# LCJebe/PCReg

Hardware: AMD Instinct MI355X
Metric: KNN Gpairs/s end-to-end (search + filters + RANSAC per step; registrations/s = 1000/ms_per_step) (higher is better)
Workload: dtype f32 (search: f16-split matrix-core candidates, exact f32 re-rank) / f64 (RANSAC)

## Files before the change

pcreg_amd/csrc/api.hip:

```cpp
#include "common.hpp"
#include <atomic>
#include <cstdarg>
#include <cmath>
#include <mutex>
#include <algorithm>
#include <vector>

namespace pcreg {

static thread_local char g_err[512] = "no error";
void set_error(const char* fmt, ...) {
    va_list ap; va_start(ap, fmt);
    vsnprintf(g_err, sizeof g_err, fmt, ap);
    va_end(ap);
}

constexpr int kKnnMaxK = PCREG_KNN_MAX_K;
constexpr int kKnnMaxQ = 4 << 20;
constexpr int kRangeMaxQ = 4 << 20;
constexpr int kScoreMaxQ = 4 << 20;
static std::mutex g_mu;
static int g_device_ok = -1;
static hipStream_t g_stream = nullptr;

// ... 39 lines not shown

}

using namespace pcreg;

#define GUARD()                                                     \
    std::lock_guard<std::mutex> lock__(g_mu);                       \
    do { int rc__ = ensure_device(); if (rc__) return rc__; } while (0)
#define TRY(expr) do { int rc__ = (expr); if (rc__) return rc__; } while (0)

namespace pcreg {
static std::atomic<int> g_debug[kDbgCount];
int debug_flag(DebugKey k) { return g_debug[k].load(std::memory_order_relaxed); }
struct Counters { DebugKey key; int n; unsigned long long* dev; };
static Counters g_match_stats{kDbgMatchStats, 8, nullptr}, g_knn_stats{kDbgKnnStats, 6, nullptr}, g_ransac_stats{kDbgRansacStats, 3, nullptr},
                g_cluster_stats{kDbgClusterStats, 4, nullptr}, g_desc_stats{kDbgDescStats, 10, nullptr},
                g_knn_direct_stats{kDbgKnnDirectStats, 3, nullptr};
static unsigned long long* counters_dev(Counters& c) {
    if (!debug_flag(c.key)) return nullptr;
    if (!c.dev) {
        if (hipMalloc((void**)&c.dev, c.n * sizeof(unsigned long long)) != hipSuccess) { c.dev = nullptr; return nullptr; }
        (void)hipMemset(c.dev, 0, c.n * sizeof(unsigned long long));
    }
    return c.dev;
}
static int counters_read(const Counters& c, long long* out, int reset, int first = 0, int count = -1) {
    PCREG_ARG(out != nullptr);
    if (count < 0) count = c.n - first;
    for (int k = 0; k < count; ++k) out[k] = 0;
    if (!c.dev) return PCREG_OK;
    PCREG_HIP(hipDeviceSynchronize());
    unsigned long long h[8];
    PCREG_HIP(hipMemcpy(h, c.dev + first, count * sizeof h[0], hipMemcpyDeviceToHost));
    for (int k = 0; k < count; ++k) out[k] = (long long)h[k];
    if (reset) PCREG_HIP(hipMemset(c.dev + first, 0, count * sizeof h[0]));
    return PCREG_OK;
}
unsigned long long* match_stats_dev() { return counters_dev(g_match_stats); }
unsigned long long* knn_stats_dev() { return counters_dev(g_knn_stats); }
unsigned long long* ransac_stats_dev() { return counters_dev(g_ransac_stats); }
unsigned long long* cluster_stats_dev() { return counters_dev(g_cluster_stats); }
unsigned long long* desc_stats_dev() { return counters_dev(g_desc_stats); }
unsigned long long* knn_direct_stats_dev() { return counters_dev(g_knn_direct_stats); }
}

extern "C" {

int pcreg_debug_set(const char* key, int value) {
    static const char* const names[pcreg::kDbgCount] = {"knn_exact", "match_exact", "match_force_fallback", "ransac_fused", "ransac_nolane",
                                                        "ransac_f64score", "ransac_resident_f64", "align_times", "align_shape", "seg_debug",
                                                        "seg_batched", "seg_wave_finalize", "match_stats", "final_batch_mb", "knn_nocull",
                                                        "knn_stats", "ransac_pass2", "ransac_stats", "range_sort_cap", "cluster_noskip",
                                                        "cluster_stats", "knn_tail_cap", "score_batch_slots", "fpfh_radius_lanes", "desc_stats",
                                                        "knn_direct", "knn_direct_stats"};
    PCREG_ARG(key != nullptr);
    for (int k = 0; k < pcreg::kDbgCount; ++k)
        if (!strcmp(key, names[k])) { pcreg::g_debug[k].store(value, std::memory_order_relaxed); return PCREG_OK; }
    pcreg::set_error("pcreg_debug_set: unknown key '%s'", key);
    return PCREG_E_ARG;
}

int pcreg_debug_match_stats(long long out[8], int reset) { return pcreg::counters_read(pcreg::g_match_stats, out, reset); }
int pcreg_debug_knn_stats(long long out[4], int reset) { return pcreg::counters_read(pcreg::g_knn_stats, out, reset, 0, 4); }
int pcreg_debug_knn_unit_stats(long long out[2], int reset) { return pcreg::counters_read(pcreg::g_knn_stats, out, reset, 4, 2); }
int pcreg_debug_knn_direct_stats(long long out[3], int reset) { return pcreg::counters_read(pcreg::g_knn_direct_stats, out, reset); }
int pcreg_debug_ransac_stats(long long out[3], int reset) { return pcreg::counters_read(pcreg::g_ransac_stats, out, reset); }
int pcreg_debug_cluster_stats(long long out[4], int reset) { return pcreg::counters_read(pcreg::g_cluster_stats, out, reset); }
int pcreg_debug_desc_stats(long long out[10], int reset) {
    PCREG_ARG(out != nullptr);
    TRY(pcreg::counters_read(pcreg::g_desc_stats, out, reset, 0, 8));
    return pcreg::counters_read(pcreg::g_desc_stats, out + 8, reset, 8, 2);
}

const char* pcreg_last_error(void) { return g_err; }
const char* pcreg_version(void) { return "pcreg-hip 0.1 (gfx950)"; }

int pcreg_device_count(int* count) {
    PCREG_ARG(count != nullptr);
    hipError_t e = hipGetDeviceCount(count);
    if (e != hipSuccess) { *count = 0; (void)hipGetLastError(); }
    return PCREG_OK;
}

static void*  g_pin[2] = {nullptr, nullptr};
static size_t g_pin_bytes[2] = {0, 0};
static hipEvent_t g_pairs_ev = nullptr;

int pcreg_set_device(int ordinal) {
    std::lock_guard<std::mutex> lock(g_mu);
    int count = 0;
    if (hipGetDeviceCount(&count) != hipSuccess || count <= 0) { set_error("no HIP device available"); (void)hipGetLastError(); return PCREG_E_NODEVICE; }
    PCREG_ARG(ordinal >= 0 && ordinal < count);
    scratch().release_all();
    if (g_stream) { (void)hipStreamDestroy(g_stream); g_stream = nullptr; }
    if (g_pairs_ev) { (void)hipEventDestroy(g_pairs_ev); g_pairs_ev = nullptr; }
    for (int k = 0; k < 2; ++k) if (g_pin[k]) { (void)hipHostFree(g_pin[k]); g_pin[k] = nullptr; g_pin_bytes[k] = 0; }
    g_device_ok = -1;
    PCREG_HIP(hipSetDevice(ordinal));
    return ensure_device();
}

int pcreg_device_name(char* buf, int cap) {
    PCREG_ARG(buf != nullptr && cap > 0);
    GUARD();
    int dev = 0; PCREG_HIP(hipGetDevice(&dev));
    hipDeviceProp_t prop; PCREG_HIP(hipGetDeviceProperties(&prop, dev));
    snprintf(buf, (size_t)cap, "%s (%s, %d CUs)", prop.name, prop.gcnArchName, prop.multiProcessorCount);
// ... 2416 lines not shown
```

pcreg_amd/csrc/common.hpp:

```cpp
#pragma once
#include <cstdlib>
#include <hip/hip_runtime.h>
#include <cstdint>
#include <cstdio>
#include <cstring>
#include <algorithm>
#include <string>
#include "../../include/pcreg.h"

namespace pcreg {

void set_error(const char* fmt, ...);
int  ensure_device();

#define PCREG_HIP(call)                                                                  \
    do {                                                                                 \
        hipError_t e__ = (call);                                                         \
        if (e__ != hipSuccess) {                                                         \
            ::pcreg::set_error("%s failed: %s (%s:%d)", #call, hipGetErrorString(e__),   \
                               __FILE__, __LINE__);                                      \
            return PCREG_E_HIP;                                                          \
        }                                                                                \
    } while (0)

// ... 2 lines not shown
        if (!(cond)) {                                                                   \
            ::pcreg::set_error("bad argument: %s (%s:%d)", #cond, __FILE__, __LINE__);   \
            return PCREG_E_ARG;                                                          \
        }                                                                                \
    } while (0)

struct Scratch {
    static constexpr int kSlots = 24;
    void*  ptr[kSlots]  = {};
    size_t size[kSlots] = {};
    int get(int slot, size_t bytes, void** out);
    void release_all();
};
Scratch& scratch();
struct Stage {
    Scratch& s; int next = 0;
    template <class T> int take(size_t count, T** out) {
        void* p = nullptr;
        const int rc = s.get(next, count * sizeof(T), &p);
        if (rc == PCREG_OK) ++next;
        *out = (T*)p;
        return rc;
    }
};

enum DebugKey {
    kDbgKnnExact = 0,
    kDbgMatchExact,
    kDbgMatchForceFallback,
    kDbgRansacFused,
    kDbgRansacNoLane,
    kDbgRansacF64Score,
    kDbgRansacResidentF64,
    kDbgAlignTimes,
    kDbgAlignShape,
    kDbgSegDebug,
    kDbgSegBatched,
    kDbgSegWaveFinalize,
    kDbgMatchStats,
    kDbgFinalBatchMB,
    kDbgKnnNoCull,
    kDbgKnnStats,
    kDbgRansacPass2,
    kDbgRansacStats,
    kDbgRangeSortCap,
    kDbgClusterNoSkip,
    kDbgClusterStats,
    kDbgKnnTailCap,
    kDbgScoreBatchSlots,
    kDbgFpfhRadiusLanes,
    kDbgDescStats,
    kDbgKnnDirect,
    kDbgKnnDirectStats,
    kDbgCount
};
int debug_flag(DebugKey k);
unsigned long long* match_stats_dev();
unsigned long long* knn_stats_dev();
unsigned long long* knn_direct_stats_dev();
unsigned long long* ransac_stats_dev();
unsigned long long* cluster_stats_dev();
unsigned long long* desc_stats_dev();
#ifdef PCREG_EXPERIMENTS
static inline int pcreg_env_int(const char* name, int dflt) { const char* e = getenv(name); return e ? atoi(e) : dflt; }
static inline const char* pcreg_env_str(const char* name) { return getenv(name); }
#define PCREG_EXP_ENV(name, dflt) pcreg_env_int(name, dflt)
#define PCREG_EXP_STR(name) pcreg_env_str(name)
#else
#define PCREG_EXP_ENV(name, dflt) (dflt)
#define PCREG_EXP_STR(name) ((const char*)nullptr)
#endif

static inline size_t align_up(size_t x, size_t a) { return (x + a - 1) / a * a; }

struct WsWalk {
    char* base; size_t off = 0;
    explicit WsWalk(void* b) : base((char*)b) {}
    void* take_bytes(size_t bytes) { void* p = base ? base + off : nullptr; off += bytes; return p; }
    template <class T> T* take(size_t count, size_t align = 256) { return (T*)take_bytes(align_up(count * sizeof(T), align)); }
    size_t bytes() const { return off; }
};

template <typename T>
static int upload_cols(const T* host, int n, int ld, int cols, T* dev, hipStream_t st) {
    if (n <= 0 || cols <= 0) return PCREG_OK;
    if (ld == n) { PCREG_HIP(hipMemcpyAsync(dev, host, sizeof(T) * (size_t)n * cols, hipMemcpyHostToDevice, st)); }
    else PCREG_HIP(hipMemcpy2DAsync(dev, sizeof(T) * (size_t)n, host, sizeof(T) * (size_t)ld, sizeof(T) * (size_t)n, cols, hipMemcpyHostToDevice, st));
    return PCREG_OK;
}

struct RansacDims { int n_cap; int iters; int B; };

size_t ransac_workspace_bytes(int iters, int B, int n_cap);
int launch_ransac(const double* p1, const double* p2, int ld, const int32_t* offsets ,
                  const int32_t* n_dev , int n_cap, int B,
                  const pcreg_ransac_opts& o, const int32_t* sample_idx_dev,
                  pcreg_dev_ransac_result* out , int32_t* inlier_idx, int32_t* iter_inl ,
                  int32_t* iter_inl_ref, void* ws, size_t ws_bytes, hipStream_t st);
int launch_ransac_partial(const double* p1, const double* p2, int ld, const int32_t* n_dev, int n_cap,
                          const pcreg_ransac_opts& o, const int32_t* sample_idx_dev, int hyp_begin, int hyp_count,
                          pcreg_dev_ransac_part* part, void* ws, size_t ws_bytes, hipStream_t st);
int launch_ransac_finish(const double* p1, const double* p2, int ld, const int32_t* n_dev, int n_cap,
                         const pcreg_ransac_opts& o, const pcreg_dev_ransac_part* combined,
                         pcreg_dev_ransac_result* out, int32_t* inlier_idx, hipStream_t st, int n_parts = 1);
int launch_estimate_transform(const double* p1, const double* p2, int n, int ld, double* T16_dev,
                              int32_t* empty_dev, hipStream_t st);
// ... 185 lines not shown
```

pcreg_amd/csrc/knn_fast.hip:

```cpp
#include "common.hpp"
#include "select.hpp"
#include "knn_fast_common.hpp"
#include <cmath>
#include <cstdlib>
#include <cstdio>
#include <algorithm>

namespace pcreg {

size_t knn_f16_prep_bytes(int M);
void knn_f16_shape(int Q, int M, int target_blocks, int* q_blocks, int* W);
int launch_prep_model_f16(const float* m, int M, int ldm, const void* prep, unsigned* rm2, void* mtiles, int32_t* seed_cnt,
                          void* seed_slots, hipStream_t st);
int launch_knn_candidates_f16(const float* q, int Q, int ldq, const int32_t* qperm, const float* dk, int M, const void* prep,
                              const void* mtiles, const float* tbox, const float* ubox, int cull, int32_t* n_vis, int32_t* vis_list, uint32_t* vis_mask, unsigned* gthr,
                              void* cand_ent, int32_t* cand_cnt, void* ctr, int target_blocks, bool dry, bool timed, const float* ug_part,
                              int ug_nparts, int ug_cells, void* ug_prep, int* W_out, hipStream_t st);

namespace {

__global__ __launch_bounds__(kBlock) void model_bbox_partial_kernel(const float* __restrict__ m, int M, int ldm,
                                                                    float* __restrict__ part ,
                                                                    int32_t* __restrict__ zero_me, int n_zero) {
    for (int i = blockIdx.x * kBlock + threadIdx.x; i < n_zero; i += gridDim.x * kBlock) zero_me[i] = 0;
// ... 97 lines not shown
__global__ __launch_bounds__(kBlock) void model_order_scatter_kernel(const float* __restrict__ m, int M, int ldm, const Prep* __restrict__ prep,
                                                                     int32_t* __restrict__ off, int32_t* __restrict__ perm, float* __restrict__ ms) {
    for (int i = blockIdx.x * kBlock + threadIdx.x; i < M; i += gridDim.x * kBlock) {
        const float x = m[i], y = m[i + (size_t)ldm], z = m[i + 2 * (size_t)ldm];
        const int d = atomicAdd(&off[sort_key(x, y, z, prep)], 1);
        perm[d] = i; ms[d] = x; ms[d + (size_t)M] = y; ms[d + 2 * (size_t)M] = z;
    }
}
__global__ __launch_bounds__(kBlock) void tile_box_kernel(const float* __restrict__ ms, int M, float* __restrict__ tbox, float* __restrict__ ubox) {
    float lo[3] = {INFINITY, INFINITY, INFINITY}, hi[3] = {-INFINITY, -INFINITY, -INFINITY};
    for (int r = threadIdx.x; r < kT16; r += kBlock) {
        const int i = blockIdx.x * kT16 + r;
        float ulo[3] = {INFINITY, INFINITY, INFINITY}, uhi[3] = {-INFINITY, -INFINITY, -INFINITY};
        if (i < M) {
#pragma unroll
            for (int c = 0; c < 3; ++c) { ulo[c] = uhi[c] = ms[i + (size_t)c * M]; lo[c] = fminf(lo[c], ulo[c]); hi[c] = fmaxf(hi[c], uhi[c]); }
        }
#pragma unroll
        for (int c = 0; c < 3; ++c) {
#pragma unroll
            for (int o = 32; o > 0; o >>= 1) { ulo[c] = fminf(ulo[c], __shfl_xor(ulo[c], o)); uhi[c] = fmaxf(uhi[c], __shfl_xor(uhi[c], o)); }
        }
        if ((threadIdx.x & 63) == 0) {
            float* ub = ubox + ((size_t)blockIdx.x * (kT16 / 64) + (size_t)(r >> 6)) * 6;
#pragma unroll
            for (int c = 0; c < 3; ++c) { ub[c] = ulo[c]; ub[3 + c] = uhi[c]; }
        }
    }
    __shared__ float s[kBlock / 64][6];
#pragma unroll
    for (int c = 0; c < 3; ++c) {
#pragma unroll
        for (int o = 32; o > 0; o >>= 1) { lo[c] = fminf(lo[c], __shfl_xor(lo[c], o)); hi[c] = fmaxf(hi[c], __shfl_xor(hi[c], o)); }
    }
    if ((threadIdx.x & 63) == 0) {
#pragma unroll
        for (int c = 0; c < 3; ++c) { s[threadIdx.x >> 6][c] = lo[c]; s[threadIdx.x >> 6][3 + c] = hi[c]; }
    }
    __syncthreads();
    if (threadIdx.x < 6) {
        float v = s[0][threadIdx.x];
        for (int w = 1; w < kBlock / 64; ++w) v = threadIdx.x < 3 ? fminf(v, s[w][threadIdx.x]) : fmaxf(v, s[w][threadIdx.x]);
        tbox[(size_t)blockIdx.x * 6 + threadIdx.x] = v;
    }
}
__global__ __launch_bounds__(kBlock) void query_order_kernel(const float* __restrict__ q, int Q, int ldq, const Prep* __restrict__ prep,
                                                             int32_t* __restrict__ off, int32_t* __restrict__ qperm) {
    const int qi = blockIdx.x * kBlock + threadIdx.x;
    if (qi >= Q) return;
    const int key = sort_key(q[qi], q[qi + (size_t)ldq], q[qi + 2 * (size_t)ldq], prep) >> 3;
    qperm[atomicAdd(&off[key], 1)] = qi;
}

__global__ __launch_bounds__(kBlock) void query_order_ranked_kernel(const float* __restrict__ q, int Q, int ldq, const Prep* __restrict__ prep,
                                                                    const int32_t* __restrict__ cnt, const int32_t* __restrict__ rank,
                                                                    int32_t* __restrict__ qperm) {
    constexpr int kPer = kQueryKeys / kBlock, kSub = kPer / 16;
    static_assert(kQueryKeys % (kBlock * 16) == 0, "every thread owns whole groups of 16 counters");
    __shared__ int s_sub[kQueryKeys / 16], s_w[kBlock / 64];
    const int lane = threadIdx.x & 63, wave = threadIdx.x >> 6;
    const int4* p = (const int4*)cnt + (size_t)threadIdx.x * (kPer / 4);
    int sub[kSub], sum = 0;
#pragma unroll
    for (int j = 0; j < kSub; ++j) {
        const int4 a = p[4 * j], b = p[4 * j + 1], c = p[4 * j + 2], d = p[4 * j + 3];
        sub[j] = sum;
        sum += (a.x + a.y + a.z + a.w) + (b.x + b.y + b.z + b.w) + (c.x + c.y + c.z + c.w) + (d.x + d.y + d.z + d.w);
    }
    int inc = sum;
#pragma unroll
    for (int o = 1; o < 64; o <<= 1) { const int y = __shfl_up(inc, o); if (lane >= o) inc += y; }
    if (lane == 63) s_w[wave] = inc;
    __syncthreads();
    int run = inc - sum;
    for (int k = 0; k < wave; ++k) run += s_w[k];
#pragma unroll
    for (int j = 0; j < kSub; ++j) s_sub[threadIdx.x * kSub + j] = run + sub[j];
    __syncthreads();
    const int qi = blockIdx.x * kBlock + threadIdx.x;
    if (qi >= Q) return;
    const int key = sort_key(q[qi], q[qi + (size_t)ldq], q[qi + 2 * (size_t)ldq], prep) >> 3;
    const int4* f = (const int4*)cnt + (size_t)(key >> 4) * 4;
    const int r = key & 15;
    int off = s_sub[key >> 4];
#pragma unroll
    for (int i = 0; i < 4; ++i) {
        const int4 v = f[i];
        off += (4 * i < r ? v.x : 0) + (4 * i + 1 < r ? v.y : 0) + (4 * i + 2 < r ? v.z : 0) + (4 * i + 3 < r ? v.w : 0);
    }
    qperm[off + rank[qi]] = qi;
}

__device__ __forceinline__ int seed_cell(float v, float lo, float inv_h, int n) {
    int c = (int)floorf((v - lo) * inv_h);
    return c < 0 ? 0 : (c >= n ? n - 1 : c);
}
constexpr int kSeedRounds = (27 + 1) / 2;
__host__ __device__ constexpr int seed_offsets(int c27) { return (c27 % 3) | (((c27 / 3) % 3) << 2) | ((c27 / 9) << 4); }
constexpr int kSeedBatch = 7;
static_assert(kSeedSlots == 4 && kSeedRounds % kSeedBatch == 0, "a quad per cell, the rounds in whole batches");
__device__ __forceinline__ void sort4(float (&d)[4]) {
#define PCREG_CS(a, b) { const float lo_ = fminf(d[a], d[b]), hi_ = fmaxf(d[a], d[b]); d[a] = lo_; d[b] = hi_; }
    PCREG_CS(0, 1) PCREG_CS(2, 3) PCREG_CS(0, 2) PCREG_CS(1, 3) PCREG_CS(1, 2)
#undef PCREG_CS
}
__global__ __launch_bounds__(kBlock, 8) void seed_query_kernel(const float* __restrict__ q, int Q, int ldq,
                                                            const Prep* __restrict__ prep, const int32_t* __restrict__ cnt,
                                                            const float4* __restrict__ slots, int seeded, unsigned* __restrict__ gthr,
                                                            int32_t* __restrict__ cand_cnt, SearchCounters* __restrict__ ctr,
                                                            float* __restrict__ ug_part, int32_t* __restrict__ ug_cnt, int ug_cells,
                                                            float* __restrict__ dk_out, int32_t* __restrict__ qcnt, int32_t* __restrict__ qrank) {
    for (int i = blockIdx.x * kBlock + threadIdx.x; i < (int)(sizeof(SearchCounters) / 4); i += gridDim.x * kBlock) ((int32_t*)ctr)[i] = 0;
    if (ug_cnt) for (int i = blockIdx.x * kBlock + threadIdx.x; i < ug_cells; i += gridDim.x * kBlock) ug_cnt[i] = 0;
    const int qi = (blockIdx.x * kBlock + threadIdx.x) >> 3, sub = threadIdx.x & 7;
    const bool live = qi < Q;
    const int qq = live ? qi : 0;
    const float qx = q[qq], qy = q[qq + (size_t)ldq], qz = q[qq + 2 * (size_t)ldq];
    if (ug_part) {
        __shared__ float s_box[kBlock / 64][6];
        float v[6] = {live ? qx : INFINITY, live ? qy : INFINITY, live ? qz : INFINITY, live ? qx : -INFINITY, live ? qy : -INFINITY, live ? qz : -INFINITY};
#pragma unroll
        for (int c = 0; c < 3; ++c) {
#pragma unroll
            for (int o = 32; o > 0; o >>= 1) { v[c] = fminf(v[c], __shfl_xor(v[c], o)); v[3 + c] = fmaxf(v[3 + c], __shfl_xor(v[3 + c], o)); }
        }
        if ((threadIdx.x & 63) == 0) {
#pragma unroll
            for (int c = 0; c < 6; ++c) s_box[threadIdx.x >> 6][c] = v[c];
        }
        __syncthreads();
        if (threadIdx.x < 6) {
            float r = s_box[0][threadIdx.x];
            for (int w = 1; w < kBlock / 64; ++w) r = threadIdx.x < 3 ? fminf(r, s_box[w][threadIdx.x]) : fmaxf(r, s_box[w][threadIdx.x]);
            ug_part[(size_t)blockIdx.x * 6 + threadIdx.x] = r;
        }
    }
    if (!seeded) {
        if (live && sub == 0) {
            cand_cnt[qi] = 0; gthr[qi] = 0xFFFFFFFFu; dk_out[qi] = INFINITY;
            if (qcnt) qrank[qi] = atomicAdd(&qcnt[sort_key(qx, qy, qz, prep) >> 3], 1);
        }
        return;
    }
    const int nx = prep->nx, ny = prep->ny, nz = prep->nz;
    const int cx = seed_cell(qx, prep->gx0, prep->inv_h, nx), cy = seed_cell(qy, prep->gy0, prep->inv_h, ny), cz = seed_cell(qz, prep->gz0, prep->inv_h, nz);
    const int quad = sub >> 2, slot = sub & 3, own = (cz * ny + cy) * nx + cx;
    int cell[kSeedRounds]; unsigned on = 0;
#pragma unroll
    for (int r = 0; r < kSeedRounds; ++r) {
        const int a = 2 * r, b = a + 1;
        const int o = quad ? seed_offsets(b) : seed_offsets(a);
        const int x = cx + (o & 3) - 1, y = cy + ((o >> 2) & 3) - 1, z = cz + (o >> 4) - 1;
        const bool ok = (b < 27 || !quad) & ((unsigned)x < (unsigned)nx) & ((unsigned)y < (unsigned)ny) & ((unsigned)z < (unsigned)nz);
        cell[r] = ok ? (z * ny + y) * nx + x : own;
        on |= (unsigned)ok << r;
    }
    const int key = sort_key(qx, qy, qz, prep) >> 3;
    int rank = 0;
    if (live && sub == 0) {
        cand_cnt[qi] = 0;
        if (qcnt) rank = atomicAdd(&qcnt[key], 1);
    }
    float d[4] = {INFINITY, INFINITY, INFINITY, INFINITY};
#pragma unroll
    for (int r0 = 0; r0 < kSeedRounds; r0 += kSeedBatch) {
        int n[kSeedBatch]; float4 pp[kSeedBatch];
#pragma unroll
        for (int t = 0; t < kSeedBatch; ++t) n[t] = cnt[cell[r0 + t]];
#pragma unroll
        for (int t = 0; t < kSeedBatch; ++t) pp[t] = slots[(size_t)cell[r0 + t] * kSeedSlots + slot];
#pragma unroll
        for (int t = 0; t < kSeedBatch; ++t) {
            const float ex = qx - pp[t].x, ey = qy - pp[t].y, ez = qz - pp[t].z;
            const float dd = __builtin_fmaf(ez, ez, __builtin_fmaf(ey, ey, ex * ex));
            const bool counts = ((on >> (r0 + t)) & 1) & (slot < min(n[t], kSeedSlots)) & (dd < d[3]);
            float c = counts ? dd : INFINITY;
#pragma unroll
            for (int k = 0; k < 4; ++k) { const float lo = fminf(d[k], c); c = fmaxf(d[k], c); d[k] = lo; }
        }
    }
#pragma unroll
    for (int o = 1; o < 8; o <<= 1) {
        float e[4];
#pragma unroll
        for (int k = 0; k < 4; ++k) e[k] = __shfl_xor(d[k], o);
#pragma unroll
        for (int k = 0; k < 4; ++k) d[k] = fminf(d[k], e[3 - k]);
        sort4(d);
    }
    if (!live || sub != 0) return;
    unsigned word = 0xFFFFFFFFu;
    const float dk = d[kSeedRank - 1];
    if (dk < INFINITY) {
        const float tx = qx - prep->cx, ty = qy - prep->cy, tz = qz - prep->cz;
        const double r2 = (double)tx * tx + (double)ty * ty + (double)tz * tz;
        const double E = score_error_bound(1, (double)prep->rm2, sqrt(r2));
        const double u = 5.9604644775390625e-08;
        const double t = (double)dk - r2 + 2.0 * E + 16.0 * u * ((double)dk + fabs((double)dk - r2));
        word = f2ord(nextafterf((float)t, INFINITY));
    }
    gthr[qi] = word;
    dk_out[qi] = dk;
    if (qcnt) qrank[qi] = rank;
}

__device__ __forceinline__ bool lex_lt_f(float da, int ia, float db, int ib) {
    return da < db || (da == db && (unsigned)ia < (unsigned)ib);
}
constexpr int LPQ = 8;
constexpr int kOwnEnt = 8;
constexpr int kEntBatch = 1;
__device__ __forceinline__ void expand_flagged(unsigned flagged, int j_own, int lane, float qx, float qy, float qz,
                                               const float* __restrict__ ms, int M, const int32_t* __restrict__ perm,
                                               float& d1, float& d2, int& i1, int& i2) {
    const int r0 = 8 * (lane >> 2) + (lane & 3);
    while (flagged) {
        int j[kEntBatch]; bool have[kEntBatch];
        float x[kEntBatch][2], y[kEntBatch][2], z[kEntBatch][2]; int oj[kEntBatch][2];
#pragma unroll
        for (int t = 0; t < kEntBatch; ++t) {
            have[t] = flagged != 0;
            const int owner = have[t] ? __builtin_ctz(flagged) : 0;
            flagged &= flagged - 1;
            j[t] = __shfl(j_own, owner, LPQ);
            if (t > 0 && !have[t]) j[t] = j[0];
#pragma unroll
            for (int h = 0; h < 2; ++h) {
                const int jj = min(j[t] + r0 + 16 * h, M - 1);
                x[t][h] = ms[jj]; y[t][h] = ms[jj + (size_t)M]; z[t][h] = ms[jj + 2 * (size_t)M]; oj[t][h] = perm[jj];
            }
        }
#pragma unroll
        for (int t = 0; t < kEntBatch; ++t) {
#pragma unroll
            for (int h = 0; h < 2; ++h) {
                const float d = point_d2(qx, qy, qz, x[t][h], y[t][h], z[t][h]);
                const bool in2 = have[t] && j[t] + r0 + 16 * h < M && lex_lt_f(d, oj[t][h], d2, i2), in1 = in2 && lex_lt_f(d, oj[t][h], d1, i1);
                d2 = in1 ? d1 : (in2 ? d : d2); i2 = in1 ? i1 : (in2 ? oj[t][h] : i2);
                d1 = in1 ? d : d1; i1 = in1 ? oj[t][h] : i1;
            }
        }
    }
}
__device__ __forceinline__ unsigned group_flags(bool f) {
    return (unsigned)(__ballot(f) >> (threadIdx.x & 63 & ~(LPQ - 1))) & ((1u << LPQ) - 1);
}
__device__ __forceinline__ void group_top2_merge(float& d1, float& d2, int& i1, int& i2) {
#pragma unroll
    for (int o = LPQ / 2; o > 0; o >>= 1) {
        float e1 = __shfl_xor(d1, o), e2 = __shfl_xor(d2, o);
        int j1 = __shfl_xor(i1, o), j2 = __shfl_xor(i2, o);
        bool first_mine = lex_lt_f(d1, i1, e1, j1);
        float w1 = first_mine ? d1 : e1; int k1 = first_mine ? i1 : j1;
        float x2 = first_mine ? d2 : d1; int y2 = first_mine ? i2 : i1;
        float x3 = first_mine ? e1 : e2; int y3 = first_mine ? j1 : j2;
        bool sec_mine = lex_lt_f(x2, y2, x3, y3);
        d1 = w1; i1 = k1; d2 = sec_mine ? x2 : x3; i2 = sec_mine ? y2 : y3;
    }
}

constexpr int kDirectBatch = 4;
constexpr int kDirectSlots = (kDirectCells + LPQ - 1) / LPQ;
__global__ __launch_bounds__(kBlock) void knn_direct_kernel(
    const float* __restrict__ q, int Q, int ldq, const float* __restrict__ dk, const Prep* __restrict__ prep,
    const int32_t* __restrict__ sort_cnt, const float* __restrict__ ms, int M, const int32_t* __restrict__ perm, int idx_base,
    int32_t* __restrict__ idx, float* __restrict__ dist, int32_t* __restrict__ cand_cnt, SearchCounters* __restrict__ ctr) {
    constexpr int kGroups = kBlock / LPQ, kTab = LPQ * kDirectSlots;
    __shared__ int s_end[kGroups][kTab], s_off[kGroups][kTab];
    __shared__ int s_n[2];
    const int lane = threadIdx.x & (LPQ - 1), grp = threadIdx.x / LPQ;
    const int qi = blockIdx.x * kGroups + grp;
    const bool live = qi < Q;
    const int qq = live ? qi : 0;
    if (threadIdx.x < 2) s_n[threadIdx.x] = 0;
    const float qx = q[qq], qy = q[qq + (size_t)ldq], qz = q[qq + 2 * (size_t)ldq], D = dk[qq];
    const float qv[3] = {qx, qy, qz}, s0[3] = {prep->sx0, prep->sy0, prep->sz0};
    DirectRange R;
    bool ok = direct_range(qv, D, s0, prep->inv_s, (1 << kSortBits) - 1, &R) && live;
    if (!ok) { for (int c = 0; c < 3; ++c) R.lo[c] = R.hi[c] = 0; }
    const int nx = R.hi[0] - R.lo[0] + 1, ny = R.hi[1] - R.lo[1] + 1;
    const int ncell = direct_cells(R);
    ok = ok && ncell <= kDirectCells;
    int e0[kDirectSlots], e1[kDirectSlots]; bool has[kDirectSlots], first[kDirectSlots];
#pragma unroll
    for (int k = 0; k < kDirectSlots; ++k) {
        const int c = lane + LPQ * k;
        has[k] = ok && c < ncell;
        const int cc = has[k] ? c : 0;
        const int ix = R.lo[0] + cc % nx, iy = R.lo[1] + (cc / nx) % ny, iz = R.lo[2] + cc / (nx * ny);
        const int key = (int)(morton_spread((unsigned)ix) | (morton_spread((unsigned)iy) << 1) | (morton_spread((unsigned)iz) << 2));
        first[k] = key == 0;
        e0[k] = sort_cnt[max(key - 1, 0)]; e1[k] = sort_cnt[key];
    }
    int total = 0;
#pragma unroll
    for (int k = 0; k < kDirectSlots; ++k) {
        const int start = first[k] ? 0 : e0[k], n = has[k] ? max(e1[k] - start, 0) : 0;
        int inc = n;
#pragma unroll
        for (int o = 1; o < LPQ; o <<= 1) { const int y = __shfl_up(inc, o, LPQ); if (lane >= o) inc += y; }
        const int end = total + inc;
        s_end[grp][lane + LPQ * k] = end;
        s_off[grp][lane + LPQ * k] = start - (end - n);
        total += __shfl(inc, LPQ - 1, LPQ);
    }
    ok = ok && total <= kDirectRows;
    const int rows = ok ? total : 0;
    __syncthreads();
    float d1 = INFINITY, d2 = INFINITY; int i1 = -1, i2 = -1;
    int c = 0;
    for (int r0 = 0; r0 < rows; r0 += LPQ * kDirectBatch) {
        float x[kDirectBatch], y[kDirectBatch], z[kDirectBatch]; int oj[kDirectBatch]; bool in[kDirectBatch];
#pragma unroll
        for (int t = 0; t < kDirectBatch; ++t) {
            const int r = r0 + LPQ * t + lane;
            in[t] = r < rows;
            const int rr = in[t] ? r : 0;
            if (in[t]) while (c < ncell - 1 && rr >= s_end[grp][c]) ++c;
            const int row = min(max(rr + s_off[grp][in[t] ? c : 0], 0), M - 1);
            x[t] = ms[row]; y[t] = ms[row + (size_t)M]; z[t] = ms[row + 2 * (size_t)M]; oj[t] = perm[row];
        }
#pragma unroll
        for (int t = 0; t < kDirectBatch; ++t) {
            const float d = point_d2(qx, qy, qz, x[t], y[t], z[t]);
            const bool in2 = in[t] && lex_lt_f(d, oj[t], d2, i2), in1 = in2 && lex_lt_f(d, oj[t], d1, i1);
            d2 = in1 ? d1 : (in2 ? d : d2); i2 = in1 ? i1 : (in2 ? oj[t] : i2);
            d1 = in1 ? d : d1; i1 = in1 ? oj[t] : i1;
        }
    }
    group_top2_merge(d1, d2, i1, i2);
    ok = ok && i2 >= 0;
    if (ok && lane == 0) {
        idx[(size_t)qi * 2] = i1 + idx_base; idx[(size_t)qi * 2 + 1] = i2 + idx_base;
        dist[(size_t)qi * 2] = d1; dist[(size_t)qi * 2 + 1] = d2;
        cand_cnt[qi] = kDirectMark;
        atomicAdd(&s_n[0], 1); atomicAdd(&s_n[1], rows);
    }
    __syncthreads();
    if (threadIdx.x == 0 && s_n[0] > 0) { atomicAdd(&ctr->n_direct, s_n[0]); atomicAdd(&ctr->direct_rows, s_n[1]); }
}

__global__ __launch_bounds__(kBlock) void knn_finalize_kernel(
    const float* __restrict__ q, int Q, int ldq, const float* __restrict__ ms, int M, const int32_t* __restrict__ perm,
    const Prep* __restrict__ prep, const unsigned* __restrict__ rm2_bits, const unsigned* __restrict__ gthr,
    const uint2* __restrict__ ent_all, const int32_t* __restrict__ cand_cnt, int cap, int idx_base,
    int32_t* __restrict__ idx, float* __restrict__ dist, int32_t* __restrict__ flag_list, int32_t* __restrict__ n_flag,
    const UgPrep* __restrict__ ug_prep, int32_t* __restrict__ ug_cnt, float4* __restrict__ ug_slots) {
    const int lane = threadIdx.x & (LPQ - 1);
    const int qi = blockIdx.x * (kBlock / LPQ) + (threadIdx.x / LPQ);
    if (qi >= Q) return;
    const float qx = q[qi], qy = q[qi + (size_t)ldq], qz = q[qi + 2 * (size_t)ldq];
    if (ug_prep && lane == 0) {
        const UgPrep P = *ug_prep;
        const int cell = (ug_cell1(qz, P.z0, P.inv_c, P.nz) * P.ny + ug_cell1(qy, P.y0, P.inv_c, P.ny)) * P.nx + ug_cell1(qx, P.x0, P.inv_c, P.nx);
        const int s = atomicAdd(&ug_cnt[cell], 1);
        if (s < kUgSlots) ug_slots[(size_t)cell * kUgSlots + s] = make_float4(qx, qy, qz, __int_as_float(qi));
    }
    const int listed = cand_cnt[qi];
    if (direct_answered(listed)) return;
    const int total = min(listed, cap);
    const uint2* ent = ent_all + (size_t)qi * cap;
    float a1 = INFINITY, a2 = INFINITY;
    uint2 own[kOwnEnt];
    const int last = max(total, 1) - 1;
#pragma unroll
    for (int k = 0; k < kOwnEnt; ++k) own[k] = ent[min(lane + LPQ * k, last)];
#pragma unroll
    for (int k = 0; k < kOwnEnt; ++k) {
        const float s = __uint_as_float(own[k].y);
        if (lane + LPQ * k < total && (int)own[k].x >= 0) { if (s < a2) { if (s < a1) { a2 = a1; a1 = s; } else a2 = s; } }
    }
    for (int e = lane + LPQ * kOwnEnt; e < total; e += LPQ) {
        const uint2 v = ent[e];
        const float s = __uint_as_float(v.y);
        if ((int)v.x >= 0) { if (s < a2) { if (s < a1) { a2 = a1; a1 = s; } else a2 = s; } }
    }
#pragma unroll
    for (int o = LPQ / 2; o > 0; o >>= 1) {
        float b1 = __shfl_xor(a1, o), b2 = __shfl_xor(a2, o);
        float n1 = fminf(a1, b1);
        float n2 = fminf(fmaxf(a1, b1), fminf(a2, b2));
        a1 = n1; a2 = n2;
    }
    const double u = 5.9604644775390625e-08;
    const float cxf = prep->cx, cyf = prep->cy, czf = prep->cz, sg = prep->sigma;
    const float tx = qx - cxf, ty = qy - cyf, tz = qz - czf;
    const bool scored = scale_usable(prep) && fabsf(sg * tx) <= kQueryScaledMax && fabsf(sg * ty) <= kQueryScaledMax && fabsf(sg * tz) <= kQueryScaledMax;
    const double r2 = (double)tx * tx + (double)ty * ty + (double)tz * tz;
    const double r = sqrt(r2);
    const double Rm2 = (double)__uint_as_float(*rm2_bits);
    const double Eab = score_error_bound(1, Rm2, r);
    const float cut = (float)((double)a2 + 2.0 * Eab + 16.0 * u * fabs((double)a2 + r2));
// ... 290 lines not shown
    int ob = (v.M + kBlock * 4 - 1) / (kBlock * 4); if (ob > 2048) ob = 2048;
    hipLaunchKernelGGL(model_order_count_kernel, dim3(ob), dim3(kBlock), 0, st, v.m, v.M, v.ldm, (const Prep*)v.prep, v.sort_cnt);
    hipLaunchKernelGGL(exclusive_scan_1wg_kernel, dim3(1), dim3(1024), 0, st, v.sort_cnt, kSortKeys);
    hipLaunchKernelGGL(model_order_scatter_kernel, dim3(ob), dim3(kBlock), 0, st, v.m, v.M, v.ldm, (const Prep*)v.prep, v.sort_cnt, v.perm, v.ms);
    PCREG_HIP(hipGetLastError());
    int rc = launch_prep_model_f16(v.ms, v.M, v.M, v.prep, v.rm2, v.tiles, v.seeded ? v.seed_cnt : nullptr, v.seed_slots, st);
    if (rc) return rc;
    hipLaunchKernelGGL(tile_box_kernel, dim3((unsigned)n_f16_tiles(v.M)), dim3(kBlock), 0, st, (const float*)v.ms, v.M, v.tbox, v.ubox);
    PCREG_HIP(hipGetLastError());
    return PCREG_OK;
}

static constexpr int kTargetBlocks = 4096;
static size_t tail_many(size_t qq) { return (size_t)(kTailGrid + (qq + kTailQ - 1) / kTailQ) * kTailQ * 2; }
SearchWs search_ws_layout(int Q, int M, void* base, size_t* bytes) {
    SearchWs s{};
    const size_t qq = (size_t)(Q > 0 ? Q : 1);
    int q_blocks, W;
    knn_f16_shape(Q > 0 ? Q : 1, M > 0 ? M : 1, kTargetBlocks, &q_blocks, &W);
    s.cap = W * KC;
    WsWalk w(base);
    s.ctr = w.take_bytes(align_up(sizeof(SearchCounters), 256));
    s.gthr = w.take<unsigned>(qq); s.flag_list = w.take<int32_t>(qq); s.cand_cnt = w.take<int32_t>(qq);
    s.cand_ent = w.take_bytes(align_up(qq * (size_t)(kF16MaxS * KC) * 8, 256));
    const size_t many = tail_many(qq);
    const size_t plan_head = align_up((size_t)q_blocks * 4, 256) / 4, plan_list = (size_t)q_blocks * std::max<size_t>(n_f16_tiles(M), 1),
                 plan = plan_head + 2 * plan_list;
    s.tail_idx = w.take<int32_t>(std::max(many, plan)); s.tail_dist = w.take<float>(many);
    s.n_vis = s.tail_idx; s.vis_list = s.tail_idx ? s.tail_idx + plan_head : nullptr;
    s.vis_mask = s.tail_idx ? (uint32_t*)(s.tail_idx + plan_head + plan_list) : nullptr;
    s.ug_cells = (int)ug_cells_cap(Q);
    s.ug_nparts = (int)((qq * 8 + kBlock - 1) / kBlock);
    s.ug_prep = w.take_bytes(256);
    s.ug_part = w.take<float>((size_t)s.ug_nparts * 6);
    s.ug_cnt = w.take<int32_t>((size_t)s.ug_cells);
    s.ug_slots = w.take_bytes(align_up((size_t)s.ug_cells * kUgSlots * 16, 256));
    s.qcnt = (int32_t*)w.take_bytes((size_t)kQueryKeys * 4);
    s.qperm = w.take<int32_t>(qq); s.dk = w.take<float>(qq);
    *bytes = w.bytes(); return s;
}
size_t search_ws_bytes(int Q, int M) { size_t b; (void)search_ws_layout(Q, M, nullptr, &b); return b; }

int launch_model_search(const ModelView& v, const float* q, int Q, int ldq, int32_t idx_base, int32_t* idx, float* dist,
                        void* ws, size_t ws_bytes, bool with_grid, bool timed, hipStream_t st) {
    PCREG_ARG(Q >= 0 && ldq >= Q && Q <= kMaxQTiles * 1024);
    if (Q == 0) return PCREG_OK;
    size_t need;
    SearchWs s = search_ws_layout(Q, v.M, ws, &need);
    if (ws_bytes < need) { set_error("search workspace too small: %zu < %zu", ws_bytes, need); return PCREG_E_WORKSPACE; }
    SearchCounters* ctr = (SearchCounters*)s.ctr;
    const bool grid = with_grid && v.M > 0;
    const bool order = v.M > 0;
    if (order) PCREG_HIP(hipMemsetAsync(s.qcnt, 0, (size_t)kQueryKeys * 4, st));
    hipLaunchKernelGGL(seed_query_kernel, dim3(s.ug_nparts), dim3(kBlock), 0, st, q, Q, ldq, (const Prep*)v.prep, (const int32_t*)v.seed_cnt,
                       (const float4*)v.seed_slots, (v.seeded && v.M > 0) ? 1 : 0, s.gthr, s.cand_cnt, ctr, grid ? s.ug_part : nullptr,
                       grid ? s.ug_cnt : nullptr, s.ug_cells, s.dk, order ? s.qcnt : nullptr, s.flag_list);
    if (v.seeded && v.M > 0 && debug_flag(kDbgKnnDirect) == 0 && debug_flag(kDbgKnnStats) == 0)
        hipLaunchKernelGGL(knn_direct_kernel, dim3((Q + kBlock / LPQ - 1) / (kBlock / LPQ)), dim3(kBlock), 0, st, q, Q, ldq, (const float*)s.dk,
                           (const Prep*)v.prep, (const int32_t*)v.sort_cnt, (const float*)v.ms, v.M, (const int32_t*)v.perm, (int)idx_base, idx, dist,
                           s.cand_cnt, ctr);
    if (unsigned long long* dstats = knn_direct_stats_dev())
        hipLaunchKernelGGL(knn_direct_stats_kernel, dim3(1), dim3(64), 0, st, (const SearchCounters*)ctr, dstats);
    if (order)
        hipLaunchKernelGGL(query_order_ranked_kernel, dim3((Q + kBlock - 1) / kBlock), dim3(kBlock), 0, st, q, Q, ldq, (const Prep*)v.prep,
                           (const int32_t*)s.qcnt, (const int32_t*)s.flag_list, s.qperm);
    int W = 1;
    const int variant = PCREG_EXP_ENV("PCREG_KNN_VARIANT", 40);
    const int target_env = PCREG_EXP_ENV("PCREG_KNN_BLOCKS", 0);
    const int cull = (debug_flag(kDbgKnnNoCull) || PCREG_EXP_ENV("PCREG_KNN_NOCULL", 0)) ? 0 : 1;
    int rc = launch_knn_candidates_f16(q, Q, ldq, s.qperm, s.dk, v.M, v.prep, v.tiles, v.tbox, v.ubox, cull, s.n_vis, s.vis_list, s.vis_mask, s.gthr, s.cand_ent, s.cand_cnt, ctr,
                                       target_env > 0 ? target_env : kTargetBlocks, variant == 41, timed, grid ? s.ug_part : nullptr,
                                       s.ug_nparts, s.ug_cells, grid ? s.ug_prep : nullptr, &W, st);
    if (rc) return rc;
    hipLaunchKernelGGL(knn_finalize_kernel, dim3((Q + kBlock / LPQ - 1) / (kBlock / LPQ)), dim3(kBlock), 0, st, q, Q, ldq, (const float*)v.ms, v.M,
                       (const int32_t*)v.perm, (const Prep*)v.prep, (const unsigned*)v.rm2, (const unsigned*)s.gthr, (const uint2*)s.cand_ent,
                       (const int32_t*)s.cand_cnt, W * KC, (int)idx_base, idx, dist, s.flag_list, &ctr->n_flag,
                       grid ? (const UgPrep*)s.ug_prep : nullptr, s.ug_cnt, (float4*)s.ug_slots);
    if (unsigned long long* stats = knn_stats_dev()) {
        const long long nominal = (long long)((Q + 511) / 512) * (long long)n_f16_tiles(v.M);
        hipLaunchKernelGGL(knn_stats_kernel, dim3(1), dim3(64), 0, st, (const SearchCounters*)ctr, nominal, stats);
    }
    if (PCREG_EXP_ENV("PCREG_KNN_DEBUG", 0)) {
        int32_t nf = 0, vis[kVisitSlots];
        PCREG_HIP(hipMemcpyAsync(&nf, &ctr->n_flag, 4, hipMemcpyDeviceToHost, st));
        PCREG_HIP(hipMemcpyAsync(vis, ctr->visited, sizeof(vis), hipMemcpyDeviceToHost, st)); PCREG_HIP(hipStreamSynchronize(st));
        long long nv = 0;
        for (int k = 0; k < kVisitSlots; ++k) nv += vis[k];
        const long long qb = (Q + 511) / 512, nt = (long long)n_f16_tiles(v.M);
        fprintf(stderr, "[pcreg] knn fast: Q=%d M=%d W=%d unproven=%d visited tile pairs=%lld of %lld (%.4f)%s\n", Q, v.M, W, nf, nv, qb * nt,
                qb * nt > 0 ? (double)nv / (double)(qb * nt) : 0.0, cull ? "" : " (culling off)");
    }
    const int dbg_cap = debug_flag(kDbgKnnTailCap);
    const int tail_cap = dbg_cap > 0 && dbg_cap < kTailList ? dbg_cap : kTailList;
    hipLaunchKernelGGL(knn_tail_kernel, dim3(kTailGrid), dim3(kBlock), 0, st, q, ldq, v.m, v.M, v.ldm, (const float*)v.ms, (const int32_t*)v.perm,
                       (const float*)v.tbox, (const float*)s.dk, (int)idx_base, (const int32_t*)s.flag_list, ctr, s.tail_idx, s.tail_dist, idx, dist, tail_cap);
    PCREG_HIP(hipGetLastError());
    return PCREG_OK;
}

int launch_query_order(const ModelView& v, const float* q, int Q, int ldq, int32_t* qcnt, int32_t* qperm, hipStream_t st) {
    hipLaunchKernelGGL(exclusive_scan_1wg_kernel, dim3(1), dim3(1024), 0, st, qcnt, kQueryKeys);
    hipLaunchKernelGGL(query_order_kernel, dim3((Q + kBlock - 1) / kBlock), dim3(kBlock), 0, st, q, Q, ldq, (const Prep*)v.prep, qcnt, qperm);
    PCREG_HIP(hipGetLastError());
    return PCREG_OK;
}

int model_export(const ModelView& v, int32_t* perm, float* sorted_soa, float* tile_box, float prep[24], hipStream_t st) {
    static_assert(sizeof(Prep) <= 24 * sizeof(float), "pcreg_debug_dev_model_export copies Prep into 24 words");
    if (prep) std::fill(prep, prep + 24, 0.0f);
    if (v.M == 0) return PCREG_OK;
    if (perm) PCREG_HIP(hipMemcpyAsync(perm, v.perm, (size_t)v.M * 4, hipMemcpyDeviceToDevice, st));
    if (sorted_soa) PCREG_HIP(hipMemcpyAsync(sorted_soa, v.ms, (size_t)v.M * 12, hipMemcpyDeviceToDevice, st));
    if (tile_box) PCREG_HIP(hipMemcpyAsync(tile_box, v.tbox, n_f16_tiles(v.M) * 24, hipMemcpyDeviceToDevice, st));
    if (prep) {
        PCREG_HIP(hipMemcpyAsync(prep, v.prep, sizeof(Prep), hipMemcpyDeviceToHost, st));
        PCREG_HIP(hipStreamSynchronize(st));
    }
    return PCREG_OK;
// ... 35 lines not shown
```

Before: 133,200.

## Fuse seed and direct KNN kernels; early-exit query ordering when all queries resolved

Merges the seeding kernel and the direct exact-KNN kernel into one launch so per-query seed results stay in registers instead of going through global memory, and saves one kernel launch. Direct-phase counters are written as per-block partials rather than global atomics. The query-ordering kernel reduces those partials and returns early when every query was resolved directly, which skips ordering work. This relies on the seed grid's per-thread layout matching the direct kernel's lanes-per-query layout, and it reuses the head of cand_ent as scratch for the partials.

After: 142,300, median of 6. 6.9% higher.

```diff
diff --git a/pcreg_amd/csrc/api.hip b/pcreg_amd/csrc/api.hip
--- a/pcreg_amd/csrc/api.hip
+++ b/pcreg_amd/csrc/api.hip
@@ -115,7 +115,7 @@
                                                         "seg_batched", "seg_wave_finalize", "match_stats", "final_batch_mb", "knn_nocull",
                                                         "knn_stats", "ransac_pass2", "ransac_stats", "range_sort_cap", "cluster_noskip",
                                                         "cluster_stats", "knn_tail_cap", "score_batch_slots", "fpfh_radius_lanes", "desc_stats",
-                                                        "knn_direct", "knn_direct_stats"};
+                                                        "knn_direct", "knn_direct_stats", "knn_seed_fused"};
     PCREG_ARG(key != nullptr);
     for (int k = 0; k < pcreg::kDbgCount; ++k)
         if (!strcmp(key, names[k])) { pcreg::g_debug[k].store(value, std::memory_order_relaxed); return PCREG_OK; }
diff --git a/pcreg_amd/csrc/common.hpp b/pcreg_amd/csrc/common.hpp
--- a/pcreg_amd/csrc/common.hpp
+++ b/pcreg_amd/csrc/common.hpp
@@ -78,6 +78,7 @@
     kDbgDescStats,
     kDbgKnnDirect,
     kDbgKnnDirectStats,
+    kDbgKnnSeedFused,
     kDbgCount
 };
 int debug_flag(DebugKey k);
diff --git a/pcreg_amd/csrc/knn_fast.hip b/pcreg_amd/csrc/knn_fast.hip
--- a/pcreg_amd/csrc/knn_fast.hip
+++ b/pcreg_amd/csrc/knn_fast.hip
@@ -173,13 +173,29 @@
     qperm[atomicAdd(&off[key], 1)] = qi;
 }
 
+constexpr int kDirectPartsAll = 2048;
 __global__ __launch_bounds__(kBlock) void query_order_ranked_kernel(const float* __restrict__ q, int Q, int ldq, const Prep* __restrict__ prep,
                                                                     const int32_t* __restrict__ cnt, const int32_t* __restrict__ rank,
-                                                                    int32_t* __restrict__ qperm) {
+                                                                    int32_t* __restrict__ qperm, const int2* __restrict__ dparts, int nparts,
+                                                                    SearchCounters* __restrict__ ctr) {
     constexpr int kPer = kQueryKeys / kBlock, kSub = kPer / 16;
     static_assert(kQueryKeys % (kBlock * 16) == 0, "every thread owns whole groups of 16 counters");
     __shared__ int s_sub[kQueryKeys / 16], s_w[kBlock / 64];
+    __shared__ int s_dir[kBlock / 64][2];
     const int lane = threadIdx.x & 63, wave = threadIdx.x >> 6;
+    if (dparts != nullptr && (nparts <= kDirectPartsAll || blockIdx.x == 0)) {
+        int nd = 0, nr = 0;
+        for (int i = threadIdx.x; i < nparts; i += kBlock) { const int2 v = dparts[i]; nd += v.x; nr += v.y; }
+#pragma unroll
+        for (int o = 32; o > 0; o >>= 1) { nd += __shfl_xor(nd, o); nr += __shfl_xor(nr, o); }
+        if (lane == 0) { s_dir[wave][0] = nd; s_dir[wave][1] = nr; }
+        __syncthreads();
+        nd = 0; nr = 0;
+#pragma unroll
+        for (int w = 0; w < kBlock / 64; ++w) { nd += s_dir[w][0]; nr += s_dir[w][1]; }
+        if (blockIdx.x == 0 && threadIdx.x == 0) { ctr->n_direct = nd; ctr->direct_rows = nr; }
+        if (nparts <= kDirectPartsAll && nd == Q) return;
+    }
     const int4* p = (const int4*)cnt + (size_t)threadIdx.x * (kPer / 4);
     int sub[kSub], sum = 0;
 #pragma unroll
@@ -225,18 +241,21 @@
     PCREG_CS(0, 1) PCREG_CS(2, 3) PCREG_CS(0, 2) PCREG_CS(1, 3) PCREG_CS(1, 2)
 #undef PCREG_CS
 }
-__global__ __launch_bounds__(kBlock, 8) void seed_query_kernel(const float* __restrict__ q, int Q, int ldq,
-                                                            const Prep* __restrict__ prep, const int32_t* __restrict__ cnt,
-                                                            const float4* __restrict__ slots, int seeded, unsigned* __restrict__ gthr,
-                                                            int32_t* __restrict__ cand_cnt, SearchCounters* __restrict__ ctr,
-                                                            float* __restrict__ ug_part, int32_t* __restrict__ ug_cnt, int ug_cells,
-                                                            float* __restrict__ dk_out, int32_t* __restrict__ qcnt, int32_t* __restrict__ qrank) {
+struct SeedOut { float qx, qy, qz, dk; int qi, rank; bool live; };
+template <bool kFused>
+__device__ __forceinline__ SeedOut seed_body(const float* __restrict__ q, int Q, int ldq,
+                                             const Prep* __restrict__ prep, const int32_t* __restrict__ cnt,
+                                             const float4* __restrict__ slots, int seeded, unsigned* __restrict__ gthr,
+                                             int32_t* __restrict__ cand_cnt, SearchCounters* __restrict__ ctr,
+                                             float* __restrict__ ug_part, int32_t* __restrict__ ug_cnt, int ug_cells,
+                                             float* __restrict__ dk_out, int32_t* __restrict__ qcnt, int32_t* __restrict__ qrank) {
     for (int i = blockIdx.x * kBlock + threadIdx.x; i < (int)(sizeof(SearchCounters) / 4); i += gridDim.x * kBlock) ((int32_t*)ctr)[i] = 0;
     if (ug_cnt) for (int i = blockIdx.x * kBlock + threadIdx.x; i < ug_cells; i += gridDim.x * kBlock) ug_cnt[i] = 0;
     const int qi = (blockIdx.x * kBlock + threadIdx.x) >> 3, sub = threadIdx.x & 7;
     const bool live = qi < Q;
     const int qq = live ? qi : 0;
     const float qx = q[qq], qy = q[qq + (size_t)ldq], qz = q[qq + 2 * (size_t)ldq];
+    SeedOut out{qx, qy, qz, INFINITY, qi, 0, live};
     if (ug_part) {
         __shared__ float s_box[kBlock / 64][6];
         float v[6] = {live ? qx : INFINITY, live ? qy : INFINITY, live ? qz : INFINITY, live ? qx : -INFINITY, live ? qy : -INFINITY, live ? qz : -INFINITY};
@@ -261,7 +280,7 @@
             cand_cnt[qi] = 0; gthr[qi] = 0xFFFFFFFFu; dk_out[qi] = INFINITY;
             if (qcnt) qrank[qi] = atomicAdd(&qcnt[sort_key(qx, qy, qz, prep) >> 3], 1);
         }
-        return;
+        return out;
     }
     const int nx = prep->nx, ny = prep->ny, nz = prep->nz;
     const int cx = seed_cell(qx, prep->gx0, prep->inv_h, nx), cy = seed_cell(qy, prep->gy0, prep->inv_h, ny), cz = seed_cell(qz, prep->gz0, prep->inv_h, nz);
@@ -279,7 +298,7 @@
     const int key = sort_key(qx, qy, qz, prep) >> 3;
     int rank = 0;
     if (live && sub == 0) {
-        cand_cnt[qi] = 0;
+        if (!kFused) cand_cnt[qi] = 0;
         if (qcnt) rank = atomicAdd(&qcnt[key], 1);
     }
     float d[4] = {INFINITY, INFINITY, INFINITY, INFINITY};
@@ -309,9 +328,10 @@
         for (int k = 0; k < 4; ++k) d[k] = fminf(d[k], e[3 - k]);
         sort4(d);
     }
-    if (!live || sub != 0) return;
+    const float dk = d[kSeedRank - 1];
+    out.dk = dk; out.rank = rank;
+    if (!live || sub != 0) return out;
     unsigned word = 0xFFFFFFFFu;
-    const float dk = d[kSeedRank - 1];
     if (dk < INFINITY) {
         const float tx = qx - prep->cx, ty = qy - prep->cy, tz = qz - prep->cz;
         const double r2 = (double)tx * tx + (double)ty * ty + (double)tz * tz;
@@ -322,7 +342,16 @@
     }
     gthr[qi] = word;
     dk_out[qi] = dk;
-    if (qcnt) qrank[qi] = rank;
+    if (!kFused && qcnt) qrank[qi] = rank;
+    return out;
+}
+__global__ __launch_bounds__(kBlock, 8) void seed_query_kernel(const float* __restrict__ q, int Q, int ldq,
+                                                            const Prep* __restrict__ prep, const int32_t* __restrict__ cnt,
+                                                            const float4* __restrict__ slots, int seeded, unsigned* __restrict__ gthr,
+                                                            int32_t* __restrict__ cand_cnt, SearchCounters* __restrict__ ctr,
+                                                            float* __restrict__ ug_part, int32_t* __restrict__ ug_cnt, int ug_cells,
+                                                            float* __restrict__ dk_out, int32_t* __restrict__ qcnt, int32_t* __restrict__ qrank) {
+    (void)seed_body<false>(q, Q, ldq, prep, cnt, slots, seeded, gthr, cand_cnt, ctr, ug_part, ug_cnt, ug_cells, dk_out, qcnt, qrank);
 }
 
 __device__ __forceinline__ bool lex_lt_f(float da, int ia, float db, int ib) {
@@ -382,19 +411,16 @@
 
 constexpr int kDirectBatch = 4;
 constexpr int kDirectSlots = (kDirectCells + LPQ - 1) / LPQ;
-__global__ __launch_bounds__(kBlock) void knn_direct_kernel(
-    const float* __restrict__ q, int Q, int ldq, const float* __restrict__ dk, const Prep* __restrict__ prep,
+template <bool kFused>
+__device__ __forceinline__ void direct_body(
+    int qi, bool live, float qx, float qy, float qz, float D, const Prep* __restrict__ prep,
     const int32_t* __restrict__ sort_cnt, const float* __restrict__ ms, int M, const int32_t* __restrict__ perm, int idx_base,
-    int32_t* __restrict__ idx, float* __restrict__ dist, int32_t* __restrict__ cand_cnt, SearchCounters* __restrict__ ctr) {
+    int32_t* __restrict__ idx, float* __restrict__ dist, int32_t* __restrict__ cand_cnt, int2* __restrict__ parts) {
     constexpr int kGroups = kBlock / LPQ, kTab = LPQ * kDirectSlots;
     __shared__ int s_end[kGroups][kTab], s_off[kGroups][kTab];
     __shared__ int s_n[2];
     const int lane = threadIdx.x & (LPQ - 1), grp = threadIdx.x / LPQ;
-    const int qi = blockIdx.x * kGroups + grp;
-    const bool live = qi < Q;
-    const int qq = live ? qi : 0;
     if (threadIdx.x < 2) s_n[threadIdx.x] = 0;
-    const float qx = q[qq], qy = q[qq + (size_t)ldq], qz = q[qq + 2 * (size_t)ldq], D = dk[qq];
     const float qv[3] = {qx, qy, qz}, s0[3] = {prep->sx0, prep->sy0, prep->sz0};
     DirectRange R;
     bool ok = direct_range(qv, D, s0, prep->inv_s, (1 << kSortBits) - 1, &R) && live;
@@ -454,11 +480,32 @@
     if (ok && lane == 0) {
         idx[(size_t)qi * 2] = i1 + idx_base; idx[(size_t)qi * 2 + 1] = i2 + idx_base;
         dist[(size_t)qi * 2] = d1; dist[(size_t)qi * 2 + 1] = d2;
-        cand_cnt[qi] = kDirectMark;
+        if (!kFused) cand_cnt[qi] = kDirectMark;
         atomicAdd(&s_n[0], 1); atomicAdd(&s_n[1], rows);
     }
+    if (kFused && live && lane == 0) cand_cnt[qi] = ok ? kDirectMark : 0;
     __syncthreads();
-    if (threadIdx.x == 0 && s_n[0] > 0) { atomicAdd(&ctr->n_direct, s_n[0]); atomicAdd(&ctr->direct_rows, s_n[1]); }
+    if (threadIdx.x == 0) parts[blockIdx.x] = make_int2(s_n[0], s_n[1]);
+}
+__global__ __launch_bounds__(kBlock) void knn_direct_kernel(
+    const float* __restrict__ q, int Q, int ldq, const float* __restrict__ dk, const Prep* __restrict__ prep,
+    const int32_t* __restrict__ sort_cnt, const float* __restrict__ ms, int M, const int32_t* __restrict__ perm, int idx_base,
+    int32_t* __restrict__ idx, float* __restrict__ dist, int32_t* __restrict__ cand_cnt, int2* __restrict__ parts) {
+    const int qi = blockIdx.x * (kBlock / LPQ) + threadIdx.x / LPQ;
+    const bool live = qi < Q;
+    const int qq = live ? qi : 0;
+    direct_body<false>(qi, live, q[qq], q[qq + (size_t)ldq], q[qq + 2 * (size_t)ldq], dk[qq], prep, sort_cnt, ms, M, perm, idx_base, idx, dist,
+                       cand_cnt, parts);
+}
+__global__ __launch_bounds__(kBlock, 8) void seed_direct_kernel(
+    const float* __restrict__ q, int Q, int ldq, const Prep* __restrict__ prep, const int32_t* __restrict__ cnt,
+    const float4* __restrict__ slots, unsigned* __restrict__ gthr, int32_t* __restrict__ cand_cnt, SearchCounters* __restrict__ ctr,
+    float* __restrict__ ug_part, int32_t* __restrict__ ug_cnt, int ug_cells, float* __restrict__ dk_out, int32_t* __restrict__ qcnt,
+    int32_t* __restrict__ qrank, const int32_t* __restrict__ sort_cnt, const float* __restrict__ ms, int M,
+    const int32_t* __restrict__ perm, int idx_base, int32_t* __restrict__ idx, float* __restrict__ dist, int2* __restrict__ parts) {
+    const SeedOut s = seed_body<true>(q, Q, ldq, prep, cnt, slots, 1, gthr, cand_cnt, ctr, ug_part, ug_cnt, ug_cells, dk_out, qcnt, qrank);
+    direct_body<true>(s.qi, s.live, s.qx, s.qy, s.qz, s.dk, prep, sort_cnt, ms, M, perm, idx_base, idx, dist, cand_cnt, parts);
+    if (s.live && (threadIdx.x & (LPQ - 1)) == 0 && qcnt) qrank[s.qi] = s.rank;
 }
 
 __global__ __launch_bounds__(kBlock) void knn_finalize_kernel(
@@ -855,18 +902,28 @@
     const bool grid = with_grid && v.M > 0;
     const bool order = v.M > 0;
     if (order) PCREG_HIP(hipMemsetAsync(s.qcnt, 0, (size_t)kQueryKeys * 4, st));
-    hipLaunchKernelGGL(seed_query_kernel, dim3(s.ug_nparts), dim3(kBlock), 0, st, q, Q, ldq, (const Prep*)v.prep, (const int32_t*)v.seed_cnt,
-                       (const float4*)v.seed_slots, (v.seeded && v.M > 0) ? 1 : 0, s.gthr, s.cand_cnt, ctr, grid ? s.ug_part : nullptr,
-                       grid ? s.ug_cnt : nullptr, s.ug_cells, s.dk, order ? s.qcnt : nullptr, s.flag_list);
-    if (v.seeded && v.M > 0 && debug_flag(kDbgKnnDirect) == 0 && debug_flag(kDbgKnnStats) == 0)
-        hipLaunchKernelGGL(knn_direct_kernel, dim3((Q + kBlock / LPQ - 1) / (kBlock / LPQ)), dim3(kBlock), 0, st, q, Q, ldq, (const float*)s.dk,
+    const bool direct = v.seeded && v.M > 0 && debug_flag(kDbgKnnDirect) == 0 && debug_flag(kDbgKnnStats) == 0;
+    const bool fused = direct && debug_flag(kDbgKnnSeedFused) == 0;
+    int2* dparts = direct ? (int2*)s.cand_ent : nullptr;
+    static_assert((size_t)kF16MaxS * KC * 8 >= sizeof(int2), "the direct phase's pairs fit the head of cand_ent");
+    if (fused)
+        hipLaunchKernelGGL(seed_direct_kernel, dim3(s.ug_nparts), dim3(kBlock), 0, st, q, Q, ldq, (const Prep*)v.prep, (const int32_t*)v.seed_cnt,
+                           (const float4*)v.seed_slots, s.gthr, s.cand_cnt, ctr, grid ? s.ug_part : nullptr, grid ? s.ug_cnt : nullptr, s.ug_cells,
+                           s.dk, s.qcnt, s.flag_list, (const int32_t*)v.sort_cnt, (const float*)v.ms, v.M, (const int32_t*)v.perm, (int)idx_base,
+                           idx, dist, dparts);
+    else
+        hipLaunchKernelGGL(seed_query_kernel, dim3(s.ug_nparts), dim3(kBlock), 0, st, q, Q, ldq, (const Prep*)v.prep, (const int32_t*)v.seed_cnt,
+                           (const float4*)v.seed_slots, (v.seeded && v.M > 0) ? 1 : 0, s.gthr, s.cand_cnt, ctr, grid ? s.ug_part : nullptr,
+                           grid ? s.ug_cnt : nullptr, s.ug_cells, s.dk, order ? s.qcnt : nullptr, s.flag_list);
+    if (direct && !fused)
+        hipLaunchKernelGGL(knn_direct_kernel, dim3(s.ug_nparts), dim3(kBlock), 0, st, q, Q, ldq, (const float*)s.dk,
                            (const Prep*)v.prep, (const int32_t*)v.sort_cnt, (const float*)v.ms, v.M, (const int32_t*)v.perm, (int)idx_base, idx, dist,
-                           s.cand_cnt, ctr);
+                           s.cand_cnt, dparts);
+    if (order)
+        hipLaunchKernelGGL(query_order_ranked_kernel, dim3((Q + kBlock - 1) / kBlock), dim3(kBlock), 0, st, q, Q, ldq, (const Prep*)v.prep,
+                           (const int32_t*)s.qcnt, (const int32_t*)s.flag_list, s.qperm, (const int2*)dparts, s.ug_nparts, ctr);
     if (unsigned long long* dstats = knn_direct_stats_dev())
         hipLaunchKernelGGL(knn_direct_stats_kernel, dim3(1), dim3(64), 0, st, (const SearchCounters*)ctr, dstats);
-    if (order)
-        hipLaunchKernelGGL(query_order_ranked_kernel, dim3((Q + kBlock - 1) / kBlock), dim3(kBlock), 0, st, q, Q, ldq, (const Prep*)v.prep,
-                           (const int32_t*)s.qcnt, (const int32_t*)s.flag_list, s.qperm);
     int W = 1;
     const int variant = PCREG_EXP_ENV("PCREG_KNN_VARIANT", 40);
     const int target_env = PCREG_EXP_ENV("PCREG_KNN_BLOCKS", 0);
```
